# hirofumi0810/tensorflow_end2end_speech_recognition

Hardware: AMD Instinct MI355X
Metric: acoustic frames/sec (train), TIMIT-shaped BLSTM-CTC (higher is better)
Workload: dtype bf16; 1 GPU; TIMIT 61-phone 5x256 BLSTM-CTC, B=16/GPU, D=120, C=62, seq_len~U{100..778}, dropout 0.2, rmsprop, train step; global_batch=16, parallelism=dp1, padded_to=own Tmax per rank

## Files before the change

### include/asr_hip.h

```cpp
#ifndef ASR_HIP_H_
#define ASR_HIP_H_

#include <stddef.h>
#include <stdint.h>

#ifdef __cplusplus
extern "C" {
#endif

typedef struct asr_handle asr_handle;
typedef void* asr_stream;

typedef enum {
  ASR_OK = 0,
  ASR_ERR_INVALID_ARG = -1,
  ASR_ERR_UNSUPPORTED = -2,
  ASR_ERR_HIP = -3,
  ASR_ERR_WORKSPACE = -4
} asr_status;

typedef enum { ASR_F32 = 0, ASR_BF16 = 1 } asr_dtype;

typedef enum {
  ASR_OPT_SGD = 0, ASR_OPT_MOMENTUM = 1, ASR_OPT_NESTEROV = 2, ASR_OPT_ADAGRAD = 3,
// ... 29 lines not shown
                     uint64_t seed, uint64_t offset, asr_stream s);
int asr_dropout_apply(asr_handle* h, int dtype, const void* in, void* out, size_t n, float keep_prob, uint64_t seed,
                      uint64_t offset, asr_stream s);
int asr_relu_bwd_drop(asr_handle* h, int dtype, const float* dout, const void* out, size_t n, float keep_prob,
                      uint64_t seed, uint64_t offset, void* dpre, asr_stream s);
int asr_colsum(asr_handle* h, int dtype, const void* a, int M, int N, int lda,
               float* out, asr_stream s);

int asr_gemm(asr_handle* h, int dtype, int out_dtype, int transA, int transB,
             int M, int N, int K, const void* A, int lda, const void* B, int ldb,
             void* C, int ldc, const float* bias, int accumulate, asr_stream s);

int asr_gemm_act(asr_handle* h, int dtype, int out_dtype, int transA, int transB,
                 int M, int N, int K, const void* A, int lda, const void* B, int ldb,
                 void* C, int ldc, const float* bias, int accumulate, int act, asr_stream s);
int asr_gemm_mul(asr_handle* h, int dtype, int transA, int transB, int M, int N, int K,
                 const void* A, int lda, const void* B, int ldb, float* C, int ldc,
                 const float* bias, int accumulate, int act, const float* mul, int ldmul, asr_stream s);
int asr_gemm_drop(asr_handle* h, int dtype, int transA, int transB, int M, int N, int K, const void* A, int lda,
                  const void* B, int ldb, float* C, int ldc, const float* bias, int accumulate, int act, float keep_prob,
                  uint64_t seed, uint64_t offset, asr_stream s);
int asr_gemm_rows(asr_handle* h, int dtype, int transA, int transB, int M, int N, int K, const void* A, int lda,
                  const void* B, int ldb, float* C, int ldc, const float* bias, int accumulate, int act,
                  const float* mul, int ldmul, float keep_prob, uint64_t seed, uint64_t offset, const int32_t* rows,
                  int num_rows, asr_stream s);
enum {
  ASR_GEMMP_ROWS_128 = 0,
  ASR_GEMMP_ROWS_256,
  ASR_GEMMP_ROWS_FULL,
  ASR_GEMMP_N
};
int asr_gemm_path_counts(asr_handle* h, unsigned long long* out, int n);
int asr_reset_gemm_path_counts(asr_handle* h);

int asr_im2col3x3(asr_handle* h, int dtype, const void* in, int N, int H, int W, int Cin, int ldp,
                  void* patches, asr_stream s);
int asr_col2im3x3(asr_handle* h, const float* dpatches, int N, int H, int W, int Cin, int ldp,
                  float* din, asr_stream s);
int asr_im2col(asr_handle* h, int dtype, const void* in_nhwc, int N, int H, int W, int Cin, int kh, int kw,
               int sh, int sw, int ldp, void* patches, asr_stream s);
int asr_col2im(asr_handle* h, const float* dpatches, int N, int H, int W, int Cin, int kh, int kw,
               int sh, int sw, int ldp, float* din_nhwc, asr_stream s);
int asr_conv3x3_prep_weights(asr_handle* h, const float* w_hwio, int Cin, int Cout, void* wt_fwd,
                             void* wt_bwd, asr_stream s);
int asr_conv3x3_fwd(asr_handle* h, const void* x, int N, int H, int W, int Cin, const void* wt_fwd,
                    const float* bias, int Cout, int relu, void* out, asr_stream s);
int asr_conv3x3_fwd_drop(asr_handle* h, const void* x, int N, int H, int W, int Cin, const void* wt_fwd,
                         const float* bias, int Cout, float keep_prob, uint64_t seed, uint64_t offset, void* out,
                         asr_stream s);
int asr_conv3x3_bwd_data(asr_handle* h, const void* dy, int N, int H, int W, int Cout,
                         const void* wt_bwd, int Cin, float* dx, asr_stream s);
int asr_conv3x3_bwd_data_relu(asr_handle* h, const void* dy, int N, int H, int W, int Cout, const void* wt_bwd, int Cin,
                              const void* act_below, float keep_prob, uint64_t seed, uint64_t offset, int use_drop,
                              void* dpre_below, asr_stream s);
int asr_conv3x3_bwd_weight(asr_handle* h, const void* x, const void* dy, int N, int H, int W,
                           int Cin, int Cout, float* dw, int accumulate, asr_stream s);
int asr_conv3x3_bwd_weight_bias(asr_handle* h, const void* x, const void* dy, int N, int H, int W,
                                int Cin, int Cout, float* dw, float* dbias, asr_stream s);
int asr_maxpool2x2_fwd(asr_handle* h, int dtype, const void* in, int N, int H, int W, int C,
                       void* out, uint8_t* argmax, asr_stream s);
int asr_maxpool2x2_fwd_drop(asr_handle* h, int dtype, const void* in, int N, int H, int W, int C, void* out,
                            uint8_t* argmax, float keep_prob, uint64_t seed, uint64_t offset, asr_stream s);
int asr_maxpool2x2_bwd(asr_handle* h, const float* dout, const uint8_t* argmax, int N, int H, int W,
                       int C, float* din, asr_stream s);
int asr_conv3x3_smallc_fwd(asr_handle* h, const void* x, int N, int H, int W, int Cin, const void* w2d,
                           const float* bias, int Cout, int relu, void* out, asr_stream s);
// ... 310 lines not shown
```

### tensorflow_end2end_speech_recognition_amd/_lib.py

```python
import ctypes as C
import os

_PKG = os.path.dirname(os.path.abspath(__file__))
LIB_PATH = os.path.join(_PKG, 'libasr_hip.so')

ASR_F32, ASR_BF16 = 0, 1
OPTIMIZER_IDS = {'sgd': 0, 'momentum': 1, 'nestrov': 2, 'adagrad': 3, 'adadelta': 4,
                 'rmsprop': 5, 'adam': 6}

_vp, _i, _f, _sz = C.c_void_p, C.c_int, C.c_float, C.c_size_t
_i64, _u64 = C.c_int64, C.c_uint64

SIGNATURES = {
    'asr_abi_version': (_i, []),
    'asr_create': (_i, [C.POINTER(_vp), _i]),
    'asr_create_ex': (_i, [C.POINTER(_vp), _i, _sz]),
    'asr_scratch_bytes': (_sz, [_vp]),
    'asr_destroy': (_i, [_vp]),
    'asr_set_xcd_skip': (_i, [_vp, _i]),
    'asr_set_gemm_tn_workgroups': (_i, [_vp, _i]),
    'asr_last_error_string': (C.c_char_p, [_vp]),
    'asr_device_info': (_i, [_vp, C.POINTER(_i), C.c_char_p, _i]),
    'asr_bt_to_tb': (_i, [_vp, _i, _vp, _vp, _i, _i, _i, _vp]),
    'asr_bt_to_tb_ld': (_i, [_vp, _i, _vp, _vp, _i, _i, _i, _i, _vp]),
# ... 45 lines not shown
    'asr_conv3x4_fwd': (_i, [_vp, _vp, _i, _i, _i, _i, _vp, _vp, _i, _i, _i, _vp, _vp]),
    'asr_conv3x4_bwd_data': (_i, [_vp, _vp, _i, _i, _i, _i, _vp, _i, _vp, _vp]),
    'asr_conv3x4_bwd_weight_bias': (_i, [_vp, _vp, _vp, _i, _i, _i, _i, _i, _vp, _vp, _vp]),
    'asr_bn_workspace_bytes': (_sz, [_i64, _i]),
    'asr_bn_stats': (_i, [_vp, _vp, _i64, _i, _f, _f, _vp, _vp, _vp, _vp, _vp]),
    'asr_bn_apply': (_i, [_vp, _i, _vp, _i, _i, _i, _i, _vp, _vp, _vp, _vp, _f, _i, _vp, _vp, _vp]),
    'asr_bn_bwd': (_i, [_vp, _i, _vp, _vp, _i, _vp, _i, _i, _i, _i, _vp, _vp, _i, _vp, _vp, _vp, _vp, _vp]),
    'asr_softmax_xent_soft': (_i, [_vp, _vp, _vp, _i, _i, _f, _vp, _vp, _vp]),
    'asr_lstm_prep_weights': (_i, [_vp, _i, _vp, _vp, _i, _i, _vp, _vp, _vp, _vp, _vp]),
    'asr_lstm_prep_layer': (_i, [_vp, _i, _i, _vp, _i, _i, _i, _vp, _vp, _vp, _vp, _vp, _vp, _vp]),
    'asr_lstm_grad_finish': (_i, [_vp, _i, _vp, _i, _i, _vp, _vp, _i, _vp]),
    'asr_gate_deinterleave': (_i, [_vp, _vp, _i, _vp, _i, _i, _i, _vp]),
    'asr_lstm_fwd': (_i, [_vp, _i, _i, _i, _i, _i, _vp, _vp, _vp, _vp, _f, _f, _vp, _vp, _vp, _vp, _vp, _vp]),
    'asr_lstm_bwd': (_i, [_vp, _i, _i, _i, _i, _i, _vp, _vp, _vp, _vp, _vp, _vp, _vp, _vp, _vp, _vp,
                          _vp, _vp]),
    'asr_lstm_bwd_ex': (_i, [_vp, _i, _i, _i, _i, _i, _vp, _vp, _vp, _vp, _vp, _vp, _vp, _vp, _f, _vp, _vp,
                             _vp, _vp]),
    'asr_gru_fwd': (_i, [_vp, _i, _i, _i, _i, _vp, _vp, _vp, _vp, _vp, _i, _vp, _vp, _vp, _vp, _vp, _vp, _vp]),
    'asr_gru_bwd': (_i, [_vp, _i, _i, _i, _i, _vp, _vp, _vp, _vp, _vp, _vp, _vp, _vp, _vp, _i, _vp, _vp, _vp, _vp]),
    'asr_check_async_errors': (_i, [_vp, C.POINTER(C.c_uint)]),
    'asr_peek_async_errors': (_i, [_vp, _vp, _vp]),
    'asr_clear_async_errors': (_i, [_vp, _vp]),
    'asr_debug_set_lstm_flags': (_i, [_i]),
    'asr_debug_set_gru_persistent': (_i, [_i]),
    'asr_cluster_tile_groups': (_i, [_i, _i, _i, _i, C.POINTER(_i), C.POINTER(_i), _i]),
    'asr_recurrence_path_counts': (_i, [_vp, C.POINTER(C.c_ulonglong)]),
    'asr_reset_recurrence_path_counts': (_i, [_vp]),
    'asr_att_path_counts': (_i, [_vp, C.POINTER(C.c_ulonglong), _i]),
    'asr_reset_att_path_counts': (_i, [_vp]),
    'asr_conv_path_counts': (_i, [_vp, C.POINTER(C.c_ulonglong), _i]),
    'asr_reset_conv_path_counts': (_i, [_vp]),
    'asr_gemm_path_counts': (_i, [_vp, C.POINTER(C.c_ulonglong), _i]),
    'asr_reset_gemm_path_counts': (_i, [_vp]),
    'asr_debug_set_cluster_cu_budget': (_i, [_i]),
    'asr_debug_placement': (_i, [_vp, _vp, _i, _i, _vp]),
    'asr_debug_poison_lds': (_i, [_vp, _vp]),
    'asr_debug_tear_probe': (_i, [_vp, _vp, C.c_uint, _i, _i, _vp, _vp]),
    'asr_ctc_workspace_bytes': (_sz, [_i, _i, _i]),
    'asr_ctc_loss': (_i, [_vp, _vp, _i, _i, _i, _vp, _vp, _vp, _i, _f, _vp, _vp, _vp, _vp, _sz, _vp]),
    'asr_ctc_greedy_decode': (_i, [_vp, _vp, _i, _i, _i, _vp, _i, _vp, _vp, _vp]),
    'asr_ctc_beam_workspace_bytes': (_sz, [_i, _i, _i, _i]),
    'asr_ctc_beam_decode': (_i, [_vp, _vp, _i, _i, _i, _vp, _i, _i, _vp, _vp, _vp, _vp, _sz, _vp]),
    'asr_softmax_rows': (_i, [_vp, _vp, _vp, _i, _i, _vp]),
    'asr_lstm_cell_fwd': (_i, [_vp] * 6 + [_i, _i, _f, _f] + [_vp] * 6),
    'asr_lstm_cell_fwd_ex': (_i, [_vp] * 6 + [_i, _i, _f, _f] + [_vp] * 5 + [_vp, _vp, _vp, _i, _vp, _i, _vp]),
    'asr_lstm_cell_gemm_ok': (_i, [_i, _i, _i, _i]),
    'asr_lstm_cell_gemm_prep': (_i, [_vp, _vp, _vp, _i, _i, _vp, _vp]),
    'asr_lstm_cell_gemm_fwd': (_i, [_vp, _vp, _i, _i, _vp, _i] + [_vp] * 4 + [_i, _i, _f, _f] + [_vp] * 5 +
                               [_vp, _vp, _vp, _i, _vp, _i, _vp]),
    'asr_lstm_cell_gemm_h_bytes': (_sz, [_i, _i]),
    'asr_lstm_cell_gemm_prep_h': (_i, [_vp, _vp, _vp, _i, _i, _vp, _vp]),
    'asr_lstm_cell_gemm_fwd_h': (_i, [_vp, _vp, _i, _i, _vp] + [_vp] * 4 + [_i, _i, _f, _f] + [_vp] * 5 +
                                 [_vp, _vp, _vp, _i, _vp, _i, _vp]),
    'asr_lstm_cell_gemm_bwd_h': (_i, [_vp, _vp, _i, _i, _i, _vp, _vp, _i, _vp]),
    'asr_lstm_cell_bwd': (_i, [_vp] * 9 + [_i, _i] + [_vp] * 5),
    'asr_lstm_cell_bwd_ex': (_i, [_vp] * 9 + [_i, _i, _f] + [_vp] * 5),
    'asr_stack_frames': (_i, [_vp, _vp, _vp, _i, _i, _i, _i, _i, _vp, _vp, _vp]),
    'asr_splice': (_i, [_vp, _vp, _vp, _i, _i, _i, _i, _i, _vp, _vp]),
    'asr_att_energy_fwd': (_i, [_vp, _vp, _vp, _vp, _i, _i, _i, _i, _vp, _vp]),
    'asr_att_energy_bwd': (_i, [_vp, _vp, _vp, _vp, _vp, _i, _i, _i, _i, _vp, _vp, _vp, _vp]),
    'asr_att_softmax_ctx_fwd': (_i, [_vp, _vp, _vp, _f, _vp, _i, _i, _i, _i, _vp, _vp, _vp, _vp]),
    'asr_att_softmax_ctx_fwd_ex': (_i, [_vp, _vp, _vp, _f, _vp, _i, _i, _i, _i, _vp, _vp, _vp, _vp, _i, _vp, _i, _vp]),
    'asr_att_softmax_ctx_bwd': (_i, [_vp, _vp, _vp, _vp, _f, _vp, _i, _i, _i, _i, _vp, _vp, _vp, _vp, _vp]),
    'asr_att_loc_energy_fwd': (_i, [_vp] * 7 + [_i, _i, _i, _i, _vp, _vp]),
    'asr_att_loc_energy_bwd': (_i, [_vp] * 8 + [_i, _i, _i, _i] + [_vp] * 6 + [_i, _vp]),
    'asr_att_decoder_fwd': (_i, [_vp, _vp, _vp]),
# ... 103 lines not shown
```

### tensorflow_end2end_speech_recognition_amd/build.py

```python
import concurrent.futures
import glob
import os
import subprocess
import sys

PKG = os.path.dirname(os.path.abspath(__file__))
CSRC = os.path.join(PKG, 'csrc')
OBJ = os.path.join(CSRC, '_obj')
LIB = os.path.join(PKG, 'libasr_hip.so')
ARCH = 'gfx950'
FLAGS = ['--offload-arch=%s' % ARCH, '-O3', '-std=c++17', '-fPIC', '-Wno-unused-value']
FILE_FLAGS = {'ctc.hip': ['-fno-slp-vectorize'], 'lstm_cluster.hip': ['-mllvm', '-amdgpu-mfma-vgpr-form']}
if os.environ.get('ASR_BUILD_ABLATE') == '1':
    FILE_FLAGS['lstm_cluster.hip'] = FILE_FLAGS['lstm_cluster.hip'] + ['-DASR_LSTM_ABLATE']


def _hipcc():
    for c in (os.environ.get('HIPCC'), '/opt/rocm/bin/hipcc', 'hipcc'):
        if c and (os.path.isabs(c) and os.path.exists(c) or not os.path.isabs(c)):
            return c
    return 'hipcc'


def _stale(target, deps):
    if not os.path.exists(target):
        return True
    t = os.path.getmtime(target)
    return any(os.path.getmtime(d) > t for d in deps)


def _compile(src, headers, force):
    obj = os.path.join(OBJ, os.path.basename(src)[:-4] + '.o')
    if force or _stale(obj, [src] + headers):
        cmd = [_hipcc()] + FLAGS + FILE_FLAGS.get(os.path.basename(src), []) + ['-c', src, '-o', obj]
        r = subprocess.run(cmd, capture_output=True, text=True)
        if r.returncode != 0:
            raise RuntimeError('hipcc failed on %s:\n%s' % (src, r.stderr[-4000:]))
    return obj


def build(force=False, verbose=True):
    os.makedirs(OBJ, exist_ok=True)
    srcs = sorted(glob.glob(os.path.join(CSRC, '*.hip')))
    headers = sorted(glob.glob(os.path.join(CSRC, '*.h'))) + \
        sorted(glob.glob(os.path.join(PKG, '..', 'include', '*.h')))
    with concurrent.futures.ThreadPoolExecutor(max_workers=min(8, len(srcs))) as ex:
        objs = list(ex.map(lambda s: _compile(s, headers, force), srcs))
# ... 13 lines not shown
```

### tensorflow_end2end_speech_recognition_amd/csrc/common.h

```cpp
#pragma once
#include <hip/hip_runtime.h>
#include <stdint.h>
#include <stdio.h>
#include <string.h>
#include "../../include/asr_hip.h"

struct asr_handle {
  int device;
  int num_cu;
  char name[128];
  char err[512];
  void* scratch;
  size_t scratch_bytes;
  size_t xch_dirty[2];
  int xch_next;
  int xcd_skip;
  int tn_wgs;
  float bptt_clip;
  unsigned long long rec_counts[6];
  unsigned long long att_counts[ASR_ATT_PATH_N];
  unsigned long long conv_counts[ASR_CONVP_N];
  unsigned long long gemm_counts[ASR_GEMMP_N];
};

#define ASR_FAIL(h, code, ...)                                  \
  do {                                                          \
    if (h) snprintf((h)->err, sizeof((h)->err), __VA_ARGS__);   \
    return (code);                                              \
  } while (0)

#define ASR_CHECK_LAUNCH(h, what)                                                   \
  do {                                                                              \
    hipError_t e_ = hipGetLastError();                                              \
    if (e_ != hipSuccess) ASR_FAIL(h, ASR_ERR_HIP, "%s: %s", what, hipGetErrorString(e_)); \
  } while (0)

typedef uint16_t bf16_t;

typedef __attribute__((ext_vector_type(8))) short bf16x8_t;
typedef __attribute__((ext_vector_type(4))) float f32x4_t;

__device__ __forceinline__ float bf16_to_f32(bf16_t v) {
  return __uint_as_float(((uint32_t)v) << 16);
}
__device__ __forceinline__ bf16_t f32_to_bf16(float f) {
  return __builtin_bit_cast(unsigned short, (__bf16)f);
}

template <typename T> struct Elem;
template <> struct Elem<float> {
  static __device__ __forceinline__ float to_f32(float v) { return v; }
  static __device__ __forceinline__ float from_f32(float v) { return v; }
};
template <> struct Elem<bf16_t> {
  static __device__ __forceinline__ float to_f32(bf16_t v) { return bf16_to_f32(v); }
// ... 81 lines not shown
```

### tensorflow_end2end_speech_recognition_amd/csrc/gemm.hip

```cpp
#include "common.h"
#include "mfma_tn.h"
#include <stdlib.h>

namespace {

static inline bool first_on_device(unsigned long long& mask) {
  int d = 0;
  (void)hipGetDevice(&d);
  const unsigned long long bit = 1ull << (d & 63);
  if (mask & bit) return false;
  mask |= bit;
  return true;
}

template <typename T> struct GT;
template <> struct GT<float> {
  static constexpr int BK = 32;
  static constexpr int VEC = 4;
};
template <> struct GT<bf16_t> {
  static constexpr int BK = 64;
  static constexpr int VEC = 8;
};

// ... 250 lines not shown
    so[i] = (unsigned)(r * LD) + ((unsigned)kv ^ nt_swz(r));
  }
  bf16x8_t ra[4], rb[4];
  auto gload = [&]() {
#pragma unroll
    for (int i = 0; i < 4; ++i) {
      ra[i] = *reinterpret_cast<const bf16x8_t*>(pa[i]);
      rb[i] = *reinterpret_cast<const bf16x8_t*>(pb[i]);
      pa[i] += BK;
      pb[i] += BK;
    }
  };
  auto sstore = [&](bf16_t* st) {
#pragma unroll
    for (int i = 0; i < 4; ++i) {
      *reinterpret_cast<bf16x8_t*>(st + so[i]) = ra[i];
      *reinterpret_cast<bf16x8_t*>(st + BM * LD + so[i]) = rb[i];
    }
  };

  f32x4_t acc[4][4];
#pragma unroll
  for (int i = 0; i < 4; ++i)
#pragma unroll
    for (int j = 0; j < 4; ++j) acc[i][j] = (f32x4_t){0.f, 0.f, 0.f, 0.f};

  const int nkt = K / BK;
  gload();
  sstore(S);
  __syncthreads();
  const int fr = lane & 15, fq = lane >> 4;
  const unsigned aoff = (unsigned)((wm * 64 + fr) * LD) + ((unsigned)(fq * 8) ^ nt_swz(fr));
  const unsigned boff = (unsigned)(BM * LD + (wn * 64 + fr) * LD) + ((unsigned)(fq * 8) ^ nt_swz(fr));
  for (int kt = 0; kt < nkt; ++kt) {
    const bf16_t* cur = S + (kt & 1) * STAGE;
    if (kt + 1 < nkt) gload();
#pragma unroll
    for (int ks = 0; ks < 2; ++ks) {
      bf16x8_t a[4], b[4];
#pragma unroll
      for (int i = 0; i < 4; ++i) a[i] = *reinterpret_cast<const bf16x8_t*>(cur + aoff + i * 16 * LD + ks * 32);
#pragma unroll
      for (int j = 0; j < 4; ++j) b[j] = *reinterpret_cast<const bf16x8_t*>(cur + boff + j * 16 * LD + ks * 32);
#pragma unroll
      for (int i = 0; i < 4; ++i)
#pragma unroll
        for (int j = 0; j < 4; ++j)
          acc[i][j] = __builtin_amdgcn_mfma_f32_16x16x32_bf16(b[j], a[i], acc[i][j], 0, 0, 0);
    }
    if (kt + 1 < nkt) sstore(S + ((kt + 1) & 1) * STAGE);
    __syncthreads();
  }
#pragma unroll
  for (int i = 0; i < 4; ++i) {
    const int mi = m0 + wm * 64 + i * 16 + fr;
    if (mi >= M) continue;
    const int m = ROWS ? rows[mi] : mi;
#pragma unroll
    for (int j = 0; j < 4; ++j) {
      const int nb = n0 + wn * 64 + j * 16 + fq * 4;
      TO* cp = C + (size_t)m * ldc + nb;
      float v[4];
#pragma unroll
      for (int r = 0; r < 4; ++r) v[r] = acc[i][j][r];
      if (bias) {
        const f32x4_t bv = *reinterpret_cast<const f32x4_t*>(bias + nb);
// ... 168 lines not shown
        *reinterpret_cast<f32x4_t*>(cp) = (f32x4_t){v[0], v[1], v[2], v[3]};
      } else {
        typedef __attribute__((ext_vector_type(4))) unsigned short us4_t;
        if (accumulate) {
          const us4_t o = *reinterpret_cast<const us4_t*>(cp);
#pragma unroll
          for (int r = 0; r < 4; ++r) v[r] += bf16_to_f32(o[r]);
        }
        if (act == 1) {
#pragma unroll
          for (int r = 0; r < 4; ++r) v[r] = fmaxf(v[r], 0.f);
        }
        *reinterpret_cast<us4_t*>(cp) = (us4_t){f32_to_bf16(v[0]), f32_to_bf16(v[1]), f32_to_bf16(v[2]), f32_to_bf16(v[3])};
      }
    }
  }
}

template <typename TO, int BM, int BN, int WM, int WN, bool ROWS = false>
static void launch_gemm_nt_big(int M, int N, int K, const void* A, int lda, const void* B, int ldb, void* C, int ldc,
                               const float* bias, int accumulate, hipStream_t st, int act, const float* mul, int ldm,
                               GemmDrop drop, const int32_t* rows = nullptr) {
  const size_t lds = (size_t)2 * (BM + BN) * (64 + 8) * sizeof(bf16_t);
  static unsigned long long attr_done = 0;
  auto k = gemm_nt_bf16_big_kernel<TO, BM, BN, WM, WN, ROWS>;
  if (first_on_device(attr_done)) {
    (void)hipFuncSetAttribute((const void*)k, hipFuncAttributeMaxDynamicSharedMemorySize, (int)lds);
  }
  const long tiles = (long)(N / BN) * ((M + BM - 1) / BM);
  hipLaunchKernelGGL(k, dim3((unsigned)tiles), dim3(WM * WN * 64), lds, st, M, N, K, (const bf16_t*)A, lda,
                     (const bf16_t*)B, ldb, (TO*)C, ldc, bias, accumulate, act, mul, ldm, drop, rows);
}

static void launch_gemm_nt_rows128(int nrows, int N, int K, const void* A, int lda, const void* B, int ldb, float* C,
                                   int ldc, const float* bias, int accumulate, hipStream_t st, int act,
                                   const float* mul, int ldm, GemmDrop drop, const int32_t* rows) {
  const size_t lds = (size_t)2 * (128 + 128) * (64 + 8) * sizeof(bf16_t);
  static unsigned long long attr_done = 0;
  auto k = gemm_nt_bf16_kernel<float, true>;
  if (first_on_device(attr_done)) {
    (void)hipFuncSetAttribute((const void*)k, hipFuncAttributeMaxDynamicSharedMemorySize, (int)lds);
  }
  const int total = (N / 128) * ((nrows + 127) / 128);
  hipLaunchKernelGGL(k, dim3(total), dim3(256), lds, st, nrows, N, K, (const bf16_t*)A, lda, (const bf16_t*)B, ldb, C,
                     ldc, bias, accumulate, act, mul, ldm, drop, rows);
}

template <typename TO>
bool try_gemm_nt_bf16(int transA, int transB, int M, int N, int K, const void* A, int lda, const void* B,
                      int ldb, void* C, int ldc, const float* bias, int accumulate, hipStream_t st, int act,
                      const float* mul, int ldm, GemmDrop drop = GemmDrop{1.f, 0, 0, 0}, const int32_t* rows = nullptr,
                      int nrows = 0, unsigned long long* counts = nullptr) {
  if (transA || !transB || K % 64 != 0 || N % 128 != 0 || M < 1024) return false;
  if (drop.use && sizeof(TO) != 4) return false;
  if (mul && (sizeof(TO) != 4 || ldm % 4 != 0 || ((uintptr_t)mul) % 16 != 0)) return false;
  if (lda % 8 != 0 || ldb % 8 != 0 || ((uintptr_t)A) % 16 != 0 || ((uintptr_t)B) % 16 != 0) return false;
  if (ldc % 4 != 0 || ((uintptr_t)C) % (4 * sizeof(TO)) != 0 || (bias && ((uintptr_t)bias) % 16 != 0)) return false;
  if (rows && (sizeof(TO) != 4 || nrows < 1 || nrows > M)) return false;
  static const int big = [] { const char* e = getenv("ASR_GEMM_NT_BIG"); return e ? atoi(e) : 1; }();
  const bool fits32 = ((size_t)(M - 1) * lda + K) * sizeof(bf16_t) < 0xFFFFFFFFull && ((size_t)(N - 1) * ldb + K) * sizeof(bf16_t) < 0xFFFFFFFFull;
  const int Mk = rows ? nrows : M;
  const long tiles256 = (long)(N / 256) * ((Mk + 255) / 256);
  const bool use_big = big && fits32 && N % 256 == 0 && (big == 2 ? Mk >= 2048 : tiles256 >= 512);
  if constexpr (sizeof(TO) == 4) {
    if (rows) {
      if (use_big)
        launch_gemm_nt_big<float, 256, 256, 2, 4, true>(Mk, N, K, A, lda, B, ldb, C, ldc, bias, accumulate, st, act, mul,
                                                         ldm, drop, rows);
      else
        launch_gemm_nt_rows128(Mk, N, K, A, lda, B, ldb, (float*)C, ldc, bias, accumulate, st, act, mul, ldm, drop, rows);
      if (counts) counts[use_big ? ASR_GEMMP_ROWS_256 : ASR_GEMMP_ROWS_128] += 1;
      return true;
    }
  }
  if (use_big) {
    launch_gemm_nt_big<TO, 256, 256, 2, 4>(M, N, K, A, lda, B, ldb, C, ldc, bias, accumulate, st, act, mul, ldm, drop);
    return true;
  }
  const size_t lds = (size_t)2 * (128 + 128) * (64 + 8) * sizeof(bf16_t);
  static unsigned long long attr_done = 0;
  if (first_on_device(attr_done)) {
    (void)hipFuncSetAttribute((const void*)gemm_nt_bf16_kernel<TO>, hipFuncAttributeMaxDynamicSharedMemorySize, (int)lds);
  }
  const int total = (N / 128) * ((M + 127) / 128);
  hipLaunchKernelGGL(gemm_nt_bf16_kernel<TO>, dim3(total), dim3(256), lds, st, M, N, K, (const bf16_t*)A, lda,
                     (const bf16_t*)B, ldb, (TO*)C, ldc, bias, accumulate, act, mul, ldm, drop, (const int32_t*)nullptr);
  return true;
}

__device__ __forceinline__ int xcd_work_index(int skip) {
  const int b = blockIdx.x, x = b & 7;
  if (x < skip) return -1;
  return (b >> 3) * (8 - skip) + (x - skip);
}
static inline unsigned xcd_grid(long work, int skip) {
  const long per = 8 - skip;
  return (unsigned)((work + per - 1) / per * 8);
}

constexpr int SK_WAVES = 8;
struct SkinnyCell {
  const float *c_prev, *h_prev, *peep, *live, *out_mask;
  float *gates, *c_raw, *c_out, *h_out, *h_raw, *cell_out, *h_out2, *cell_out2;
// ... 525 lines not shown
      lda < (transA ? M : K) || ldb < (transB ? K : N) || ldc != N || N % 4 != 0 || !(keep_prob > 0.f && keep_prob <= 1.f))
    ASR_FAIL(h, ASR_ERR_INVALID_ARG, "asr_gemm_drop: bad args M=%d N=%d K=%d ldc=%d (ldc == N, N %% 4 == 0)", M, N, K, ldc);
  if (M == 0 || N == 0) return ASR_OK;
  hipStream_t st = (hipStream_t)s;
  bool fused = false;
  const GemmDrop drop = {keep_prob, seed, offset, 1};
  if (dtype == ASR_F32)
    launch_gemm<float, float>(h, transA, transB, M, N, K, A, lda, B, ldb, C, ldc, bias, accumulate, st, act, nullptr, 0, &fused, drop);
  else
    launch_gemm<bf16_t, float>(h, transA, transB, M, N, K, A, lda, B, ldb, C, ldc, bias, accumulate, st, act, nullptr, 0, &fused, drop);
  ASR_CHECK_LAUNCH(h, "asr_gemm_drop");
  if (!fused) return asr_dropout_apply(h, ASR_F32, C, C, (size_t)M * N, keep_prob, seed, offset, s);
  return ASR_OK;
}

extern "C" int asr_gemm_rows(asr_handle* h, int dtype, int transA, int transB, int M, int N, int K, const void* A,
                             int lda, const void* B, int ldb, float* C, int ldc, const float* bias, int accumulate,
                             int act, const float* mul, int ldmul, float keep_prob, uint64_t seed, uint64_t offset,
                             const int32_t* rows, int num_rows, asr_stream s) {
  if (!h) return ASR_ERR_INVALID_ARG;
  const bool use_drop = keep_prob != 0.f;
  if (!rows || num_rows < 0 || num_rows > M || (mul && use_drop))
    ASR_FAIL(h, ASR_ERR_INVALID_ARG, "asr_gemm_rows: bad row list (rows=%p num_rows=%d M=%d) or both mul and dropout",
             (const void*)rows, num_rows, M);
  if (!asr_dtype_ok(dtype) || (act != 0 && act != 1) || M < 0 || N < 0 || K < 0 || !A || !B || !C ||
      lda < (transA ? M : K) || ldb < (transB ? K : N) || ldc < N || (mul && ldmul < N) ||
      (use_drop && (ldc != N || N % 4 != 0 || !(keep_prob > 0.f && keep_prob <= 1.f))))
    ASR_FAIL(h, ASR_ERR_INVALID_ARG, "asr_gemm_rows: bad args M=%d N=%d K=%d lda=%d ldb=%d ldc=%d ldmul=%d keep_prob=%g",
             M, N, K, lda, ldb, ldc, ldmul, (double)keep_prob);
  if (M == 0 || N == 0 || num_rows == 0) return ASR_OK;
  if (dtype == ASR_BF16) {
    const GemmDrop drop = {use_drop ? keep_prob : 1.f, seed, offset, use_drop ? 1 : 0};
    if (try_gemm_nt_bf16<float>(transA, transB, M, N, K, A, lda, B, ldb, C, ldc, bias, accumulate, (hipStream_t)s, act,
                                mul, ldmul, drop, rows, num_rows, h->gemm_counts)) {
      ASR_CHECK_LAUNCH(h, "asr_gemm_rows");
      return ASR_OK;
    }
  }
  h->gemm_counts[ASR_GEMMP_ROWS_FULL] += 1;
  if (use_drop)
    return asr_gemm_drop(h, dtype, transA, transB, M, N, K, A, lda, B, ldb, C, ldc, bias, accumulate, act, keep_prob, seed,
                         offset, s);
  return asr_gemm_mul(h, dtype, transA, transB, M, N, K, A, lda, B, ldb, C, ldc, bias, accumulate, act, mul, ldmul, s);
}

extern "C" int asr_gemm_path_counts(asr_handle* h, unsigned long long* out, int n) {
  if (!h || !out || n < 0) return ASR_ERR_INVALID_ARG;
  for (int i = 0; i < n; ++i) out[i] = i < ASR_GEMMP_N ? h->gemm_counts[i] : 0ull;
  return ASR_OK;
}
extern "C" int asr_reset_gemm_path_counts(asr_handle* h) {
  if (!h) return ASR_ERR_INVALID_ARG;
  for (int i = 0; i < ASR_GEMMP_N; ++i) h->gemm_counts[i] = 0;
  return ASR_OK;
}

extern "C" int asr_lstm_cell_gemm_prep(asr_handle* h, const float* W, const float* bias, int K, int U, float* W_il,
                                       asr_stream s) {
  if (!h) return ASR_ERR_INVALID_ARG;
  if (!W || !W_il || K < 1 || U < 1 || ((uintptr_t)W_il) % 16 != 0)
    ASR_FAIL(h, ASR_ERR_INVALID_ARG, "asr_lstm_cell_gemm_prep: bad args");
  const size_t n = (size_t)(K + (bias ? 1 : 0)) * U;
  size_t blocks = (n + 255) / 256;
  if (blocks > 4096) blocks = 4096;
  hipLaunchKernelGGL(interleave_gates_kernel, dim3((unsigned)blocks), dim3(256), 0, (hipStream_t)s, W, bias, K, U, W_il);
  ASR_CHECK_LAUNCH(h, "asr_lstm_cell_gemm_prep");
  return ASR_OK;
}
extern "C" int asr_lstm_cell_gemm_ok(int B, int K, int U, int ldx) {
  return B >= 1 && B <= 32 && K >= 64 && K % 64 == 0 && U >= 8 && U % 8 == 0 && ldx % 4 == 0 && ldx >= K;
}
extern "C" int asr_lstm_cell_gemm_fwd(asr_handle* h, const float* x, int ldx, int K, const float* W_il, int has_bias,
                                      const float* c_prev, const float* h_prev, const float* peep, const float* live,
                                      int B, int U, float forget_bias, float cell_clip, float* gates, float* c_raw,
                                      float* c_out, float* h_out, float* h_raw, const float* out_mask, float* cell_out,
                                      float* h_out2, int ld_h2, float* cell_out2, int ld_c2, asr_stream s) {
  if (!h) return ASR_ERR_INVALID_ARG;
  if (!x || !W_il || !c_prev || !h_prev || !live || !gates || !c_raw || !c_out || !h_out || !h_raw ||
      !asr_lstm_cell_gemm_ok(B, K, U, ldx) || ((uintptr_t)x) % 16 != 0 || ((uintptr_t)W_il) % 16 != 0 ||
      (h_out2 && ld_h2 < U) || (cell_out2 && ld_c2 < U))
    ASR_FAIL(h, ASR_ERR_INVALID_ARG, "asr_lstm_cell_gemm_fwd: bad args (B <= 32, K %% 64 == 0, U %% 8 == 0, 16-byte aligned rows)");
  SkinnyCell c;
  c.c_prev = c_prev; c.h_prev = h_prev; c.peep = peep; c.live = live; c.out_mask = out_mask;
  c.gates = gates; c.c_raw = c_raw; c.c_out = c_out; c.h_out = h_out; c.h_raw = h_raw;
  c.cell_out = cell_out; c.h_out2 = h_out2; c.cell_out2 = cell_out2;
  c.U = U; c.ld_h2 = ld_h2; c.ld_c2 = ld_c2; c.fb = forget_bias; c.clip = cell_clip;
// ... 64 lines not shown
```

### tensorflow_end2end_speech_recognition_amd/ops.py

```python
import ctypes as C
import os
import time as _time

import numpy as np
import torch

from . import _lib
from ._lib import ASR_BF16, ASR_F32

TORCH_DTYPE = {ASR_F32: torch.float32, ASR_BF16: torch.bfloat16}


def dtype_id(dtype):
    if dtype in (ASR_F32, 'f32', 'fp32', 'float32', torch.float32):
        return ASR_F32
    if dtype in (ASR_BF16, 'bf16', 'bfloat16', torch.bfloat16):
        return ASR_BF16
    raise ValueError('dtype must be f32 or bf16, got %r' % (dtype,))


_lane = 0
_side = {}


# ... 1198 lines not shown
def conv_path_counts(device=0):
    n = len(_CONV_PATH_KEYS)
    tot = [0] * n
    for h in _device_handles(device):
        out = (C.c_ulonglong * n)()
        h.check(h.lib.asr_conv_path_counts(h.h, out, n), 'asr_conv_path_counts')
        tot = [a + int(b) for a, b in zip(tot, out)]
    return dict(zip(_CONV_PATH_KEYS, tot))


def reset_conv_path_counts(device=0):
    for h in _device_handles(device):
        h.check(h.lib.asr_reset_conv_path_counts(h.h), 'asr_reset_conv_path_counts')


_GEMM_PATH_KEYS = ('rows_128', 'rows_256', 'rows_full')


def gemm_path_counts(device=0):
    n = len(_GEMM_PATH_KEYS)
    tot = [0] * n
    for h in _device_handles(device):
        out = (C.c_ulonglong * n)()
        h.check(h.lib.asr_gemm_path_counts(h.h, out, n), 'asr_gemm_path_counts')
        tot = [a + int(b) for a, b in zip(tot, out)]
    return dict(zip(_GEMM_PATH_KEYS, tot))


def reset_gemm_path_counts(device=0):
    for h in _device_handles(device):
        h.check(h.lib.asr_reset_gemm_path_counts(h.h), 'asr_reset_gemm_path_counts')


def debug_set_cluster_cu_budget(n):
    _lib.load().asr_debug_set_cluster_cu_budget(int(n))


def debug_set_gru_persistent(on):
    _lib.load().asr_debug_set_gru_persistent(int(bool(on)))


def ctc_loss(logits, labels_flat, label_offsets, seq_len, max_label_len, grad_scale=1.0,
             want_grad=True):
    h = _h(logits)
    _chk(logits, torch.float32, 'logits')
    _chk(labels_flat, torch.int32, 'labels_flat')
    _chk(label_offsets, torch.int32, 'label_offsets')
    _chk(seq_len, torch.int32, 'seq_len')
    T, B, Cc = logits.shape
    dev = logits.device
    nbytes = h.lib.asr_ctc_workspace_bytes(T, B, int(max_label_len))
    ws = torch.empty((nbytes,), dtype=torch.uint8, device=dev)
    loss = torch.empty((B,), dtype=torch.float32, device=dev)
    grad = torch.empty_like(logits) if want_grad else None
    ninf = torch.empty((1,), dtype=torch.int32, device=dev)
    h.check(h.lib.asr_ctc_loss(h.h, _p(logits), T, B, Cc, _p(labels_flat), _p(label_offsets),
                               _p(seq_len), int(max_label_len), float(grad_scale), _p(loss), _p(grad),
                               _p(ninf), _p(ws), nbytes, _s()), 'asr_ctc_loss')
    return loss, grad, ninf


def ctc_greedy_decode(logits, seq_len, blank=None):
    h = _h(logits)
    _chk(logits, torch.float32, 'logits')
    _chk(seq_len, torch.int32, 'seq_len')
    T, B, Cc = logits.shape
# ... 466 lines not shown
```

Before: 735,000 frames/s.

## Add multi-stage async global-to-LDS pipelined kernel for row-gathered NT GEMM

Adds a new 512-thread row-gathered NT GEMM kernel for the 128x128 tile path. It loads straight from global memory into LDS with global_load_lds and uses a ring of 2 or 3 stages with counted vmcnt waits. The depth is picked from the tile count relative to the CU count. The aim is to hide global load latency and drop the register round trip and padded-LDS stores of the old double-buffered kernel. It is enabled by default via an env-var mode and also adds ablation variants and pipe-depth counters; the risks are more LDS per block and hand-written waitcnt correctness.

After: 740,600 frames/s (median of 6 runs). Within noise of the previous version (+0.8%).

```diff
diff --git a/include/asr_hip.h b/include/asr_hip.h
--- a/include/asr_hip.h
+++ b/include/asr_hip.h
@@ -85,6 +85,8 @@
 };
 int asr_gemm_path_counts(asr_handle* h, unsigned long long* out, int n);
 int asr_reset_gemm_path_counts(asr_handle* h);
+int asr_gemm_nt_pipe_counts(asr_handle* h, unsigned long long* out, int n);
+int asr_reset_gemm_nt_pipe_counts(asr_handle* h);
 
 int asr_im2col3x3(asr_handle* h, int dtype, const void* in, int N, int H, int W, int Cin, int ldp,
                   void* patches, asr_stream s);
diff --git a/tensorflow_end2end_speech_recognition_amd/_lib.py b/tensorflow_end2end_speech_recognition_amd/_lib.py
--- a/tensorflow_end2end_speech_recognition_amd/_lib.py
+++ b/tensorflow_end2end_speech_recognition_amd/_lib.py
@@ -101,6 +101,8 @@
     'asr_reset_conv_path_counts': (_i, [_vp]),
     'asr_gemm_path_counts': (_i, [_vp, C.POINTER(C.c_ulonglong), _i]),
     'asr_reset_gemm_path_counts': (_i, [_vp]),
+    'asr_gemm_nt_pipe_counts': (_i, [_vp, C.POINTER(C.c_ulonglong), _i]),
+    'asr_reset_gemm_nt_pipe_counts': (_i, [_vp]),
     'asr_debug_set_cluster_cu_budget': (_i, [_i]),
     'asr_debug_placement': (_i, [_vp, _vp, _i, _i, _vp]),
     'asr_debug_poison_lds': (_i, [_vp, _vp]),
diff --git a/tensorflow_end2end_speech_recognition_amd/build.py b/tensorflow_end2end_speech_recognition_amd/build.py
--- a/tensorflow_end2end_speech_recognition_amd/build.py
+++ b/tensorflow_end2end_speech_recognition_amd/build.py
@@ -13,6 +13,7 @@
 FILE_FLAGS = {'ctc.hip': ['-fno-slp-vectorize'], 'lstm_cluster.hip': ['-mllvm', '-amdgpu-mfma-vgpr-form']}
 if os.environ.get('ASR_BUILD_ABLATE') == '1':
     FILE_FLAGS['lstm_cluster.hip'] = FILE_FLAGS['lstm_cluster.hip'] + ['-DASR_LSTM_ABLATE']
+    FILE_FLAGS['gemm.hip'] = ['-DASR_GEMM_ABLATE']
 
 
 def _hipcc():
diff --git a/tensorflow_end2end_speech_recognition_amd/csrc/common.h b/tensorflow_end2end_speech_recognition_amd/csrc/common.h
--- a/tensorflow_end2end_speech_recognition_amd/csrc/common.h
+++ b/tensorflow_end2end_speech_recognition_amd/csrc/common.h
@@ -21,6 +21,7 @@
   unsigned long long att_counts[ASR_ATT_PATH_N];
   unsigned long long conv_counts[ASR_CONVP_N];
   unsigned long long gemm_counts[ASR_GEMMP_N];
+  unsigned long long gemm_pipe_count[2];
 };
 
 #define ASR_FAIL(h, code, ...)                                  \
diff --git a/tensorflow_end2end_speech_recognition_amd/csrc/gemm.hip b/tensorflow_end2end_speech_recognition_amd/csrc/gemm.hip
--- a/tensorflow_end2end_speech_recognition_amd/csrc/gemm.hip
+++ b/tensorflow_end2end_speech_recognition_amd/csrc/gemm.hip
@@ -306,6 +306,34 @@
   const int fr = lane & 15, fq = lane >> 4;
   const unsigned aoff = (unsigned)((wm * 64 + fr) * LD) + ((unsigned)(fq * 8) ^ nt_swz(fr));
   const unsigned boff = (unsigned)(BM * LD + (wn * 64 + fr) * LD) + ((unsigned)(fq * 8) ^ nt_swz(fr));
+#ifdef ASR_GEMM_ABLATE
+  const int abl = ROWS ? act >> 8 : 0;
+  act &= 0xff;
+  if (abl) {
+    if (abl == 2 && nkt > 1) gload();
+    for (int kt = 0; kt < nkt; ++kt) {
+      const bf16_t* cur = S + (abl == 2 ? (kt & 1) * STAGE : 0);
+      if (abl == 2 && kt + 1 < nkt) {
+        sstore(S + ((kt + 1) & 1) * STAGE);
+        if (kt + 2 < nkt) gload();
+      }
+#pragma unroll
+      for (int ks = 0; ks < 2; ++ks) {
+        bf16x8_t a[4], b[4];
+#pragma unroll
+        for (int i = 0; i < 4; ++i) a[i] = *reinterpret_cast<const bf16x8_t*>(cur + aoff + i * 16 * LD + ks * 32);
+#pragma unroll
+        for (int j = 0; j < 4; ++j) b[j] = *reinterpret_cast<const bf16x8_t*>(cur + boff + j * 16 * LD + ks * 32);
+#pragma unroll
+        for (int i = 0; i < 4; ++i)
+#pragma unroll
+          for (int j = 0; j < 4; ++j)
+            acc[i][j] = __builtin_amdgcn_mfma_f32_16x16x32_bf16(b[j], a[i], acc[i][j], 0, 0, 0);
+      }
+      __syncthreads();
+    }
+  } else
+#endif
   for (int kt = 0; kt < nkt; ++kt) {
     const bf16_t* cur = S + (kt & 1) * STAGE;
     if (kt + 1 < nkt) gload();
@@ -540,25 +568,182 @@
                      (const bf16_t*)B, ldb, (TO*)C, ldc, bias, accumulate, act, mul, ldm, drop, rows);
 }
 
-static void launch_gemm_nt_rows128(int nrows, int N, int K, const void* A, int lda, const void* B, int ldb, float* C,
-                                   int ldc, const float* bias, int accumulate, hipStream_t st, int act,
-                                   const float* mul, int ldm, GemmDrop drop, const int32_t* rows) {
+template <int D>
+__global__ __launch_bounds__(512) void gemm_nt_rows_pipe_kernel(int M, int N, int K, const bf16_t* __restrict__ A,
+                                                                int lda, const bf16_t* __restrict__ Bt, int ldb,
+                                                                float* __restrict__ C, int ldc,
+                                                                const float* __restrict__ bias, int accumulate, int act,
+                                                                const float* __restrict__ mul, int ldm, GemmDrop drop,
+                                                                const int32_t* __restrict__ rows) {
+  static_assert(D >= 2 && D <= 4, "the counted waits below are written for two to four stages");
+  constexpr int BM = 128, BN = 128, BK = 64, ROWB = BK * (int)sizeof(bf16_t);
+  constexpr int STAGE = (BM + BN) * ROWB;
+  typedef __attribute__((address_space(3))) void* lds_ptr_t;
+  typedef const __attribute__((address_space(1))) void* glb_ptr_t;
+  extern __shared__ __attribute__((aligned(16))) char smem[];
+
+  const int tid = threadIdx.x, lane = tid & 63, wave = tid >> 6;
+  const int wm = wave >> 2, wn = wave & 3;
+  const int ntn = N / BN, ntm = (M + BM - 1) / BM, total = ntn * ntm;
+  const int t = nt_tile_of_block<true>((int)blockIdx.x, total);
+  const int m0 = (t / ntn) * BM, n0 = (t % ntn) * BN;
+  const int fr = lane & 15, fq = lane >> 4;
+
+  int mrow[4];
+#pragma unroll
+  for (int i = 0; i < 4; ++i) mrow[i] = rows[min(m0 + wm * 64 + i * 16 + fr, M - 1)];
+
+  const char* src[4];
+#pragma unroll
+  for (int i = 0; i < 4; ++i) {
+    const int r = (i * 8 + wave) * 8 + (lane >> 3), kv = ((lane & 7) ^ ((r >> 1) & 7)) * 8;
+    if (i < 2)
+      src[i] = reinterpret_cast<const char*>(A + (size_t)rows[min(m0 + r, M - 1)] * lda + kv);
+    else
+      src[i] = reinterpret_cast<const char*>(Bt + (size_t)(n0 + r - BM) * ldb + kv);
+  }
+  auto issue = [&](int stage) {
+#pragma unroll
+    for (int i = 0; i < 4; ++i) {
+      __builtin_amdgcn_global_load_lds((glb_ptr_t)src[i], (lds_ptr_t)(smem + stage * STAGE + (i * 8 + wave) * 1024), 16, 0, 0);
+      src[i] += ROWB;
+    }
+  };
+
+  f32x4_t acc[4][2];
+#pragma unroll
+  for (int i = 0; i < 4; ++i)
+#pragma unroll
+    for (int j = 0; j < 2; ++j) acc[i][j] = (f32x4_t){0.f, 0.f, 0.f, 0.f};
+
+  const int nkt = K / BK;
+#pragma unroll
+  for (int i = 0; i < 4; ++i) asm volatile("" ::"v"(mrow[i]));
+#pragma unroll
+  for (int s = 0; s < D - 1; ++s)
+    if (s < nkt) issue(s);
+  const unsigned aoff = (unsigned)((wm * 64 + fr) * ROWB), boff = (unsigned)((BM + wn * 32 + fr) * ROWB);
+  const unsigned ko0 = (unsigned)((fq ^ (fr >> 1)) * 16), ko1 = (unsigned)(((4 + fq) ^ (fr >> 1)) * 16);
+  int cs = 0, ls = D - 1;
+  for (int kt = 0; kt < nkt; ++kt) {
+    const int ahead = min(D - 2, nkt - 1 - kt);
+    if (ahead >= 2) asm volatile("s_waitcnt vmcnt(8)" ::: "memory");
+    else if (ahead == 1) asm volatile("s_waitcnt vmcnt(4)" ::: "memory");
+    else asm volatile("s_waitcnt vmcnt(0)" ::: "memory");
+    __builtin_amdgcn_s_waitcnt(0xc07f);
+    asm volatile("" ::: "memory");
+    __builtin_amdgcn_s_barrier();
+    asm volatile("" ::: "memory");
+    if (kt + D - 1 < nkt) issue(ls);
+    const char* cur = smem + cs * STAGE;
+    bf16x8_t a[2][4], b[2][2];
+#pragma unroll
+    for (int ks = 0; ks < 2; ++ks) {
+      const unsigned ko = ks ? ko1 : ko0;
+#pragma unroll
+      for (int j = 0; j < 2; ++j) b[ks][j] = *reinterpret_cast<const bf16x8_t*>(cur + boff + j * 16 * ROWB + ko);
+#pragma unroll
+      for (int i = 0; i < 4; ++i) a[ks][i] = *reinterpret_cast<const bf16x8_t*>(cur + aoff + i * 16 * ROWB + ko);
+      if (ks == 0) __builtin_amdgcn_s_waitcnt(0xc07f);
+      __builtin_amdgcn_sched_barrier(0);
+    }
+#pragma unroll
+    for (int ks = 0; ks < 2; ++ks)
+#pragma unroll
+      for (int i = 0; i < 4; ++i)
+#pragma unroll
+        for (int j = 0; j < 2; ++j)
+          acc[i][j] = __builtin_amdgcn_mfma_f32_16x16x32_bf16(b[ks][j], a[ks][i], acc[i][j], 0, 0, 0);
+    cs = cs + 1 == D ? 0 : cs + 1;
+    ls = ls + 1 == D ? 0 : ls + 1;
+  }
+#pragma unroll
+  for (int i = 0; i < 4; ++i) {
+    if (m0 + wm * 64 + i * 16 + fr >= M) continue;
+    const int m = mrow[i];
+#pragma unroll
+    for (int j = 0; j < 2; ++j) {
+      const int nb = n0 + wn * 32 + j * 16 + fq * 4;
+      float* cp = C + (size_t)m * ldc + nb;
+      float v[4];
+#pragma unroll
+      for (int r = 0; r < 4; ++r) v[r] = acc[i][j][r];
+      if (bias) {
+        const f32x4_t bv = *reinterpret_cast<const f32x4_t*>(bias + nb);
+#pragma unroll
+        for (int r = 0; r < 4; ++r) v[r] += bv[r];
+      }
+      if (accumulate) {
+        const f32x4_t o = *reinterpret_cast<const f32x4_t*>(cp);
+#pragma unroll
+        for (int r = 0; r < 4; ++r) v[r] += o[r];
+      }
+      if (act == 1) {
+#pragma unroll
+        for (int r = 0; r < 4; ++r) v[r] = fmaxf(v[r], 0.f);
+      }
+      if (mul) {
+        const f32x4_t mv = *reinterpret_cast<const f32x4_t*>(mul + (size_t)m * ldm + nb);
+#pragma unroll
+        for (int r = 0; r < 4; ++r) v[r] *= mv[r];
+      }
+      if (drop.use) {
+        float mk[4];
+        asr_dropout_words(drop.offset + ((size_t)m * N + nb) / 4, drop.seed, drop.keep, 1.f / drop.keep, mk);
+#pragma unroll
+        for (int r = 0; r < 4; ++r) v[r] *= mk[r];
+      }
+      *reinterpret_cast<f32x4_t*>(cp) = (f32x4_t){v[0], v[1], v[2], v[3]};
+    }
+  }
+}
+
+static int gemm_nt_pipe_mode() {
+  static const int mode = [] { const char* e = getenv("ASR_GEMM_NT_PIPE"); return e ? atoi(e) : 1; }();
+  return mode;
+}
+
+static int launch_gemm_nt_rows128(int nrows, int N, int K, const void* A, int lda, const void* B, int ldb, float* C,
+                                  int ldc, const float* bias, int accumulate, hipStream_t st, int act,
+                                  const float* mul, int ldm, GemmDrop drop, const int32_t* rows) {
+  const int total = (N / 128) * ((nrows + 127) / 128);
+  const int mode = gemm_nt_pipe_mode();
+  if (mode == 1) {
+    static unsigned long long attr_done[2] = {0, 0}, cu_known = 0;
+    static int num_cu[64];
+    int dev = 0;
+    (void)hipGetDevice(&dev);
+    if (first_on_device(cu_known))
+      (void)hipDeviceGetAttribute(&num_cu[dev & 63], hipDeviceAttributeMultiprocessorCount, dev);
+    const int depth = total <= num_cu[dev & 63] ? 3 : 2;
+    const size_t lds = (size_t)depth * (128 + 128) * 64 * sizeof(bf16_t);
+    auto k = depth == 3 ? gemm_nt_rows_pipe_kernel<3> : gemm_nt_rows_pipe_kernel<2>;
+    if (first_on_device(attr_done[depth - 2])) {
+      (void)hipFuncSetAttribute((const void*)k, hipFuncAttributeMaxDynamicSharedMemorySize, (int)lds);
+    }
+    hipLaunchKernelGGL(k, dim3(total), dim3(512), lds, st, nrows, N, K, (const bf16_t*)A, lda, (const bf16_t*)B, ldb, C,
+                       ldc, bias, accumulate, act, mul, ldm, drop, rows);
+    return depth;
+  }
+#ifdef ASR_GEMM_ABLATE
+  act |= mode >= 2 ? (mode - 1) << 8 : 0;
+#endif
   const size_t lds = (size_t)2 * (128 + 128) * (64 + 8) * sizeof(bf16_t);
   static unsigned long long attr_done = 0;
   auto k = gemm_nt_bf16_kernel<float, true>;
   if (first_on_device(attr_done)) {
     (void)hipFuncSetAttribute((const void*)k, hipFuncAttributeMaxDynamicSharedMemorySize, (int)lds);
   }
-  const int total = (N / 128) * ((nrows + 127) / 128);
   hipLaunchKernelGGL(k, dim3(total), dim3(256), lds, st, nrows, N, K, (const bf16_t*)A, lda, (const bf16_t*)B, ldb, C,
                      ldc, bias, accumulate, act, mul, ldm, drop, rows);
+  return 0;
 }
 
 template <typename TO>
 bool try_gemm_nt_bf16(int transA, int transB, int M, int N, int K, const void* A, int lda, const void* B,
                       int ldb, void* C, int ldc, const float* bias, int accumulate, hipStream_t st, int act,
                       const float* mul, int ldm, GemmDrop drop = GemmDrop{1.f, 0, 0, 0}, const int32_t* rows = nullptr,
-                      int nrows = 0, unsigned long long* counts = nullptr) {
+                      int nrows = 0, unsigned long long* counts = nullptr, unsigned long long* pipe_count = nullptr) {
   if (transA || !transB || K % 64 != 0 || N % 128 != 0 || M < 1024) return false;
   if (drop.use && sizeof(TO) != 4) return false;
   if (mul && (sizeof(TO) != 4 || ldm % 4 != 0 || ((uintptr_t)mul) % 16 != 0)) return false;
@@ -575,8 +760,10 @@
       if (use_big)
         launch_gemm_nt_big<float, 256, 256, 2, 4, true>(Mk, N, K, A, lda, B, ldb, C, ldc, bias, accumulate, st, act, mul,
                                                          ldm, drop, rows);
-      else
-        launch_gemm_nt_rows128(Mk, N, K, A, lda, B, ldb, (float*)C, ldc, bias, accumulate, st, act, mul, ldm, drop, rows);
+      else if (const int depth = launch_gemm_nt_rows128(Mk, N, K, A, lda, B, ldb, (float*)C, ldc, bias, accumulate, st, act,
+                                                        mul, ldm, drop, rows)) {
+        if (pipe_count) pipe_count[0] += 1, pipe_count[1] += depth == 2;
+      }
       if (counts) counts[use_big ? ASR_GEMMP_ROWS_256 : ASR_GEMMP_ROWS_128] += 1;
       return true;
     }
@@ -1168,7 +1355,7 @@
   if (dtype == ASR_BF16) {
     const GemmDrop drop = {use_drop ? keep_prob : 1.f, seed, offset, use_drop ? 1 : 0};
     if (try_gemm_nt_bf16<float>(transA, transB, M, N, K, A, lda, B, ldb, C, ldc, bias, accumulate, (hipStream_t)s, act,
-                                mul, ldmul, drop, rows, num_rows, h->gemm_counts)) {
+                                mul, ldmul, drop, rows, num_rows, h->gemm_counts, h->gemm_pipe_count)) {
       ASR_CHECK_LAUNCH(h, "asr_gemm_rows");
       return ASR_OK;
     }
@@ -1188,6 +1375,16 @@
 extern "C" int asr_reset_gemm_path_counts(asr_handle* h) {
   if (!h) return ASR_ERR_INVALID_ARG;
   for (int i = 0; i < ASR_GEMMP_N; ++i) h->gemm_counts[i] = 0;
+  return ASR_OK;
+}
+extern "C" int asr_gemm_nt_pipe_counts(asr_handle* h, unsigned long long* out, int n) {
+  if (!h || !out || n < 0) return ASR_ERR_INVALID_ARG;
+  for (int i = 0; i < n; ++i) out[i] = i < 2 ? h->gemm_pipe_count[i] : 0ull;
+  return ASR_OK;
+}
+extern "C" int asr_reset_gemm_nt_pipe_counts(asr_handle* h) {
+  if (!h) return ASR_ERR_INVALID_ARG;
+  h->gemm_pipe_count[0] = h->gemm_pipe_count[1] = 0;
   return ASR_OK;
 }
 
diff --git a/tensorflow_end2end_speech_recognition_amd/ops.py b/tensorflow_end2end_speech_recognition_amd/ops.py
--- a/tensorflow_end2end_speech_recognition_amd/ops.py
+++ b/tensorflow_end2end_speech_recognition_amd/ops.py
@@ -1254,6 +1254,20 @@
         h.check(h.lib.asr_reset_gemm_path_counts(h.h), 'asr_reset_gemm_path_counts')
 
 
+def gemm_nt_pipe_counts(device=0, by_ring=False):
+    tot = [0, 0]
+    for h in _device_handles(device):
+        out = (C.c_ulonglong * 2)()
+        h.check(h.lib.asr_gemm_nt_pipe_counts(h.h, out, 2), 'asr_gemm_nt_pipe_counts')
+        tot = [a + int(b) for a, b in zip(tot, out)]
+    return tuple(tot) if by_ring else tot[0]
+
+
+def reset_gemm_nt_pipe_counts(device=0):
+    for h in _device_handles(device):
+        h.check(h.lib.asr_reset_gemm_nt_pipe_counts(h.h), 'asr_reset_gemm_nt_pipe_counts')
+
+
 def debug_set_cluster_cu_budget(n):
     _lib.load().asr_debug_set_cluster_cu_budget(int(n))
 
```
